# zkMIPS/zkm

Measured on AMD Instinct MI355X. Metric: segment_proofs_per_sec, higher is better.
Workload: dtype u64 (Goldilocks p = 2^64 - 2^32 + 1, integer modular)

## Files before the change

### zkm_amd/csrc/core.hip

```cpp
#include <sched.h>
#include <time.h>
#include <stdio.h>
#include <algorithm>
#include <atomic>

#include "poseidon_dev.h"
#include "zkm_internal.h"

void* zkm_ctx::alloc(size_t bytes) {
    if (bytes == 0) bytes = 8;
    void* p = nullptr;
    {
        std::lock_guard<std::mutex> g(alloc_mu);
        auto it = free_blocks.find(bytes);
        if (it != free_blocks.end()) {
            p = it->second;
            free_blocks.erase(it);
            live_blocks[p] = bytes;
            return p;
        }
    }
    zkm_ctx* const root = parent ? parent : this;
    const int ticket = root->debug_fail_allocs.load(std::memory_order_relaxed) > 0 ? root->debug_fail_allocs.fetch_sub(1) : 0;
    const bool inject = ticket > 0;
// ... 41 lines not shown
}
void zkm_ctx::drop_copy_streams() {
    hipStream_t a, b, d;
    {
        std::lock_guard<std::mutex> g(alloc_mu);
        a = copy_stream; b = copy_stream2; d = side_stream;
        copy_stream = copy_stream2 = side_stream = nullptr;
    }
    for (hipStream_t st : {a, b, d})
        if (st) { (void)hipStreamSynchronize(st); (void)hipStreamDestroy(st); }
}
static hipStream_t ensure_stream(zkm_ctx* c, hipStream_t& cs) {
    if (!cs) {
        hipStream_t st = nullptr;
        ZKM_HIP_CHECK(hipStreamCreateWithFlags(&st, hipStreamNonBlocking));
        std::lock_guard<std::mutex> g(c->alloc_mu);
        cs = st;
    }
    return cs;
}
hipStream_t zkm_ctx::ensure_copy_stream(int k) { return ensure_stream(this, k ? copy_stream2 : copy_stream); }
hipStream_t zkm_ctx::ensure_side_stream() { return ensure_stream(this, side_stream); }
void zkm_ctx::trim() {
    trim_self();
    shrink_down();
    drop_copy_streams();
    for (zkm_ctx* l : lanes) {
        l->trim_self();
        l->shrink_down();
        l->drop_copy_streams();
    }
}
static hipError_t zkm_stream_create(hipStream_t* st, int num_cus, int part_k, int part_n) {
    if (part_n > 1 && part_k >= 0 && part_k < part_n && num_cus >= 8 * part_n) {
        std::vector<uint32_t> mask((size_t)(num_cus + 31) / 32, 0);
        const int lo = (int)((long)num_cus * part_k / part_n), hi = (int)((long)num_cus * (part_k + 1) / part_n);
        for (int i = lo; i < hi; i++) mask[i / 32] |= 1u << (i % 32);
        return hipExtStreamCreateWithCUMask(st, (uint32_t)mask.size(), mask.data());
    }
    return hipStreamCreateWithFlags(st, hipStreamNonBlocking);
}
void zkm_ctx::ensure_lanes(size_t k) {
    while (lanes.size() < k) {
        zkm_ctx* l = new zkm_ctx();
        l->parent = this;
        l->device = device;
        l->num_cus = num_cus;
        l->ingest_chunk_cols = ingest_chunk_cols;
        l->keccak_parts_max_points = keccak_parts_max_points;
        l->fri_fused_division_min = fri_fused_division_min;
        l->wide_max_hashes = wide_max_hashes;
        l->leaf_mfma = leaf_mfma;
        l->quad_max_hashes = quad_max_hashes;
        l->small_ntt = small_ntt;
        l->tree_tail = tree_tail;
        l->commit_lanes = commit_lanes;
        l->max_stack = max_stack;
        l->fri_scan_combine = fri_scan_combine;
        l->pow_round_log = pow_round_log;
        l->cu_part_k = cu_part_k;
        l->cu_part_n = cu_part_n;
        hipError_t e = zkm_stream_create(&l->stream, num_cus, cu_part_k, cu_part_n);
        if (e != hipSuccess) {
            delete l;
            ZKM_HIP_CHECK(e);
        }
        lanes.push_back(l);
    }
    for (zkm_ctx* l : lanes) l->profiling = profiling;
}
void zkm_ctx::release(void* p) {
    if (!p) return;
    std::lock_guard<std::mutex> g(alloc_mu);
    auto it = live_blocks.find(p);
    if (it == live_blocks.end()) return;
    free_blocks.emplace(it->second, p);
    live_blocks.erase(it);
}
uint64_t* zkm_ctx::staging(size_t words) {
    if (words > h_staging_words) {
        if (h_staging) (void)hipHostFree(h_staging);
        size_t w = words < 4096 ? 4096 : words;
        ZKM_HIP_CHECK(hipHostMalloc((void**)&h_staging, w * sizeof(uint64_t)));
        h_staging_words = w;
    }
    return h_staging;
}
struct down_args {
    const uint32_t* src[4];
    uint32_t* dst[4];
    uint32_t words[4];
    uint32_t n;
};
__global__ __launch_bounds__(1024) void k_download(down_args a, uint64_t* flag, uint64_t seq) {
    for (uint32_t s = 0; s < a.n; s++)
        for (uint32_t i = threadIdx.x; i < a.words[s]; i += 1024) a.dst[s][i] = a.src[s][i];
    __threadfence_system();
    __syncthreads();
    if (threadIdx.x == 0) __hip_atomic_store(flag, seq, __ATOMIC_RELEASE, __HIP_MEMORY_SCOPE_SYSTEM);
}
__global__ __launch_bounds__(256) void k_download_wide(const uint4* __restrict__ src, uint4* __restrict__ dst, uint32_t n16, uint64_t* flag,
                                                       uint64_t seq, unsigned* counter) {
    for (uint32_t i = blockIdx.x * 256 + threadIdx.x; i < n16; i += gridDim.x * 256) dst[i] = src[i];
    __threadfence_system();
    __syncthreads();
    if (threadIdx.x == 0) {
// ... 257 lines not shown
        if (!out) throw std::runtime_error("zkm_ctx_create: null argument");
        int n = 0;
        ZKM_HIP_CHECK(hipGetDeviceCount(&n));
        if (device < 0 || device >= n) throw std::runtime_error("zkm_ctx_create: no such HIP device " + std::to_string(device));
        ZKM_HIP_CHECK(hipSetDevice(device));
        std::unique_ptr<zkm_ctx> c(new zkm_ctx());
        c->device = device;
        hipDeviceProp_t prop;
        ZKM_HIP_CHECK(hipGetDeviceProperties(&prop, device));
        c->num_cus = prop.multiProcessorCount;
        if (const char* part = getenv("ZKM_CU_MASK_PART")) {
            int k = -1, n = 0;
            if (sscanf(part, "%d/%d", &k, &n) == 2) { c->cu_part_k = k; c->cu_part_n = n; }
        }
        ZKM_HIP_CHECK(zkm_stream_create(&c->stream, c->num_cus, c->cu_part_k, c->cu_part_n));
        g_live_contexts.fetch_add(1, std::memory_order_relaxed);
        *out = c.release();
    });
}

void zkm_ctx_destroy(zkm_ctx* c) {
    if (!c) return;
    if (!c->parent) g_live_contexts.fetch_sub(1, std::memory_order_relaxed);
    (void)hipSetDevice(c->device);
    for (zkm_ctx* l : c->lanes) zkm_ctx_destroy(l);
    c->lanes.clear();
    (void)hipStreamSynchronize(c->stream);
    if (c->copy_stream) { (void)hipStreamSynchronize(c->copy_stream); (void)hipStreamDestroy(c->copy_stream); }
    if (c->copy_stream2) { (void)hipStreamSynchronize(c->copy_stream2); (void)hipStreamDestroy(c->copy_stream2); }
    if (c->side_stream) { (void)hipStreamSynchronize(c->side_stream); (void)hipStreamDestroy(c->side_stream); }
    for (auto& kv : c->free_blocks) (void)hipFree(kv.second);
    for (auto& kv : c->live_blocks) (void)hipFree(kv.first);
    for (auto& r : c->prof) { (void)hipEventDestroy(r.start); (void)hipEventDestroy(r.stop); }
    for (auto e : c->event_pool) (void)hipEventDestroy(e);
    if (c->h_staging) (void)hipHostFree(c->h_staging);
    if (c->h_xfer) (void)hipHostFree(c->h_xfer);
    if (c->h_down) (void)hipHostFree(c->h_down);
    if (c->block_event) (void)hipEventDestroy(c->block_event);
    (void)hipStreamDestroy(c->stream);
    delete c;
}

int zkm_ctx_set_tuning(zkm_ctx* c, const char* key, uint64_t value, char** err) {
    return zkm_api("zkm_ctx_set_tuning", err, [&] {
        if (!c || !key) throw std::runtime_error("zkm_ctx_set_tuning: null argument");
        const std::string k(key);
        auto set = [&](zkm_ctx* x) {
            if (k == "ingest_chunk_cols") x->ingest_chunk_cols = (size_t)value;
            else if (k == "keccak_parts_max_points") x->keccak_parts_max_points = (size_t)value;
            else if (k == "fri_fused_division_min") x->fri_fused_division_min = (size_t)value;
            else if (k == "wide_max_hashes") x->wide_max_hashes = (size_t)value;
            else if (k == "leaf_mfma") x->leaf_mfma = value ? 1 : 0;
            else if (k == "quad_max_hashes") x->quad_max_hashes = (size_t)value;
            else if (k == "block_after_us") x->block_after_us = value;
            else if (k == "small_ntt") x->small_ntt = value ? 1 : 0;
            else if (k == "tree_tail") x->tree_tail = value ? 1 : 0;
            else if (k == "pow_round_log") x->pow_round_log = value < 8 ? 8 : (value > 22 ? 22 : (unsigned)value);
            else if (k == "fri_scan_combine") x->fri_scan_combine = value ? 1 : 0;
            else if (k == "aux_pipeline") x->aux_pipeline = value ? 1 : 0;
            else if (k == "commit_lanes") x->commit_lanes = value < 1 ? 1 : (value > 8 ? 8 : (size_t)value);
            else if (k == "segments_memory_budget") x->segments_memory_budget = (size_t)value;
            else if (k == "max_stack") x->max_stack = value < 1 ? 1 : (value > ZKM_MAX_SEG ? ZKM_MAX_SEG : (size_t)value);
            else if (k == "throughput_profile") {
                x->commit_lanes = value ? 1 : ZKM_COMMIT_LANES;
                x->wide_max_hashes = value ? 256 : 1024;
                x->quad_max_hashes = value ? 4096 : 32768;
                x->pow_round_log = value ? 16 : 17;
            }
            else if (k == "check_ctls") x->check_ctls = value ? 1 : 0;
            else if (k == "verify") x->verify = value ? 1 : 0;
            else if (k == "boot_chain_quad") x->boot_chain_quad = value ? 1 : 0;
            else if (k == "debug_verify_flip") {
                const char* hooks = getenv("ZKM_ENABLE_TEST_HOOKS");
                if (!hooks || strcmp(hooks, "1") != 0) throw std::runtime_error("zkm_ctx_set_tuning: unknown key '" + k + "'");
                x->debug_verify_flip = value;
            }
            else if (k == "debug_ctl_key_bits") {
                const char* hooks = getenv("ZKM_ENABLE_TEST_HOOKS");
                if (!hooks || strcmp(hooks, "1") != 0) throw std::runtime_error("zkm_ctx_set_tuning: unknown key '" + k + "'");
                x->debug_ctl_key_bits = value > 128 ? 128 : (unsigned)value;
            }
            else if (k == "debug_fail_allocs") {
                const char* hooks = getenv("ZKM_ENABLE_TEST_HOOKS");
                if (!hooks || strcmp(hooks, "1") != 0) throw std::runtime_error("zkm_ctx_set_tuning: unknown key '" + k + "'");
                if (x == c) x->debug_fail_allocs.store((int)value);
            }
            else throw std::runtime_error("zkm_ctx_set_tuning: unknown key '" + k + "'");
        };
        set(c);
        for (zkm_ctx* l : c->lanes) set(l);
    });
}

uint64_t zkm_ctx_host_waits(const zkm_ctx* c) { return c ? c->host_waits : 0; }

int zkm_ctx_synchronize(zkm_ctx* c, char** err) {
    return zkm_api("zkm_ctx_synchronize", c, err, [&] { c->sync(); });
}
void* zkm_ctx_stream(zkm_ctx* c) { return c ? (void*)c->stream : nullptr; }

void zkm_ctx_memory(const zkm_ctx* c, size_t* live_bytes, size_t* cached_bytes) {
    size_t live = 0, cached = 0;
    if (c) {
        for (auto& kv : c->live_blocks) live += kv.second;
        for (auto& kv : c->free_blocks) cached += kv.first;
        for (const zkm_ctx* l : c->lanes) {
// ... 324 lines not shown
    gl_t* __restrict__ d = dst + (size_t)blockIdx.y * words;
    for (size_t i = (size_t)blockIdx.x * 256 + threadIdx.x; i < words; i += (size_t)gridDim.x * 256) d[i] = gl_canon(s[i]);
}

void zkm_launch_canon(zkm_ctx* c, gl_t* v, size_t total) {
    zkm_prof_scope ps(c, "ingest_canonicalise");
    hipLaunchKernelGGL(k_canon, dim3((total + 255) / 256), dim3(256), 0, c->stream, v, total);
    ZKM_HIP_CHECK(hipGetLastError());
}

void zkm_batch_build(zkm_batch* b, const uint64_t* src, bool src_is_values, gl_t* dev_values, const uint64_t* const* src_cols,
                     const uint64_t* const* seg_srcs) {
    zkm_ctx* c = b->ctx;
    const size_t nseg = b->nseg;
    size_t n = b->n(), N = b->N(), ncols = b->ncols * nseg;
    if (b->log_n + b->rate_bits > 30) throw std::runtime_error("polynomial batch too large");
    if (nseg == 0 || nseg > ZKM_MAX_SEG) throw std::runtime_error("polynomial batch: bad segment count");
    if (ncols > 65535 && nseg > 1) throw std::runtime_error("polynomial batch: too many stacked columns");
    if (!src && !src_cols && !seg_srcs) throw std::runtime_error("polynomial batch: no source");
    if (src_cols)
        for (size_t i = 0; i < ncols; i++)
            if (!src_cols[i]) throw std::runtime_error("polynomial batch: null column pointer");
    if (seg_srcs)
        for (size_t i = 0; i < nseg; i++)
            if (!seg_srcs[i]) throw std::runtime_error("polynomial batch: null segment pointer");
    auto copy_cols = [&](gl_t* dst, size_t c0, size_t nc, hipMemcpyKind kind, hipStream_t st) {
        if (seg_srcs) {
            for (size_t sg = 0; sg < nseg; sg++)
                ZKM_HIP_CHECK(hipMemcpyAsync(dst + sg * b->ncols * n, seg_srcs[sg], b->ncols * n * sizeof(gl_t), hipMemcpyDefault, st));
            return;
        }
        if (!src_cols) {
            ZKM_HIP_CHECK(hipMemcpyAsync(dst, src + c0 * n, nc * n * sizeof(gl_t), kind, st));
            return;
        }
        for (size_t i = 0; i < nc; i++)
            ZKM_HIP_CHECK(hipMemcpyAsync(dst + i * n, src_cols[c0 + i], n * sizeof(gl_t), hipMemcpyDefault, st));
    };
    b->coeffs = (gl_t*)c->alloc(ncols * n * sizeof(gl_t));
    b->lde = (gl_t*)c->alloc(ncols * N * sizeof(gl_t));
    b->coeff_s1 = b->rate_bits == 2 ? zkm_coeff_layout_s1(b->log_n) : 0;
    const unsigned s1 = b->coeff_s1;
    auto inverse_transform = [&](const gl_t* vals, size_t c0, size_t nc) {
        if (s1) zkm_intt_digit(c, vals, n, b->coeffs + c0 * n, n, nc, b->log_n);
        else zkm_ntt_natural_ex(c, vals, n, b->lde + c0 * N, n, b->coeffs + c0 * n, n, nc, b->log_n, true, 0);
    };
    size_t dwords = zkm_merkle_layout(b->lde_bits(), b->cap_height, b->level_off);
    b->dig_words = dwords;
    b->digests = (gl_t*)c->alloc(nseg * dwords * sizeof(gl_t));
    bool dev = !src_cols && !seg_srcs && zkm_is_device_ptr(src);
    hipMemcpyKind kind = dev ? hipMemcpyDeviceToDevice : hipMemcpyHostToDevice;
    const size_t CH = c->ingest_chunk_cols;
    bool leaves_done = false;
    if (src_is_values && !dev && nseg == 1 && CH && CH % 8 == 0 && ncols >= 2 * CH && b->log_n >= 13) {
        c->ensure_copy_stream();
        const size_t nchunks = (ncols + CH - 1) / CH;
        zkm_scratch state(c, 12 * N * sizeof(gl_t));
        std::vector<zkm_event> ev;
        ev.reserve(nchunks + 1);
        struct drain {
            zkm_ctx* c;
            ~drain() {
                (void)hipStreamSynchronize(c->copy_stream);
                (void)hipStreamSynchronize(c->stream);
            }
        } const drained{c};
        ev.emplace_back(c);
        ev[0].record(c->stream);
        ZKM_HIP_CHECK(hipStreamWaitEvent(c->copy_stream, ev[0].e, 0));
        for (size_t k = 0; k < nchunks; k++) {
            size_t c0 = k * CH, nc = std::min(CH, ncols - c0);
            gl_t* dst = dev_values ? dev_values + c0 * n : b->lde + c0 * N;
            copy_cols(dst, c0, nc, hipMemcpyHostToDevice, c->copy_stream);
            ev.emplace_back(c);
            ev.back().record(c->copy_stream);
        }
        for (size_t k = 0; k < nchunks; k++) {
            size_t c0 = k * CH, nc = std::min(CH, ncols - c0);
            gl_t* vals = dev_values ? dev_values + c0 * n : b->lde + c0 * N;
            ZKM_HIP_CHECK(hipStreamWaitEvent(c->stream, ev[k + 1].e, 0));
            if (dev_values) zkm_launch_canon(c, vals, nc * n);
            inverse_transform(vals, c0, nc);
            zkm_lde_bitrev(c, b->coeffs + c0 * n, b->lde + c0 * N, nc, b->log_n, b->rate_bits, GL_GENERATOR, s1);
            zkm_launch_merkle_leaves_chunk(c, b->lde + c0 * N, N, nc, N, state.as<gl_t>(), k == 0, k + 1 == nchunks, b->digests);
        }
        leaves_done = true;
    } else if (src_is_values && dev) {
        inverse_transform(src, 0, ncols);
    } else if (src_is_values) {
        gl_t* vals = dev_values ? dev_values : b->lde;
        bool all_dev = seg_srcs != nullptr;
        for (size_t sg = 0; all_dev && sg < nseg; sg++) all_dev = zkm_is_device_ptr(seg_srcs[sg]);
        if (all_dev && !dev_values) {
            for (size_t sg = 0; sg < nseg; sg++) inverse_transform(seg_srcs[sg], sg * b->ncols, b->ncols);
        } else if (all_dev) {
            seg_ptrs sp{};
            for (size_t sg = 0; sg < nseg; sg++) sp.p[sg] = seg_srcs[sg];
            const size_t words = b->ncols * n;
            zkm_prof_scope ps(c, "ingest_canonicalise");
            hipLaunchKernelGGL(k_gather_canon, dim3((unsigned)std::min<size_t>((words + 255) / 256, 4096), (unsigned)nseg), dim3(256), 0, c->stream, sp,
                               words, vals);
            ZKM_HIP_CHECK(hipGetLastError());
        } else {
            copy_cols(vals, 0, ncols, kind, c->stream);
            if (dev_values) zkm_launch_canon(c, vals, ncols * n);
        }
        if (!(all_dev && !dev_values)) inverse_transform(vals, 0, ncols);
    } else {
        copy_cols(b->coeffs, 0, ncols, kind, c->stream);
    }
    if (!leaves_done) {
        zkm_lde_bitrev(c, b->coeffs, b->lde, ncols, b->log_n, b->rate_bits, GL_GENERATOR, src_is_values ? s1 : 0);
        zkm_launch_merkle_leaves(c, b->lde, N, b->ncols, N, b->digests, nseg, b->lde_seg(), dwords);
    }
    if (!src_is_values && s1) {
        zkm_scratch nat(c, ncols * n * sizeof(gl_t));
        ZKM_HIP_CHECK(hipMemcpyAsync(nat.p, b->coeffs, ncols * n * sizeof(gl_t), hipMemcpyDeviceToDevice, c->stream));
        zkm_coeff_layout_convert(c, nat.as<gl_t>(), n, b->coeffs, n, ncols, b->log_n, false);
    }
    size_t capw = (size_t)4 << b->cap_height;
    b->cap.resize(nseg * capw);
    zkm_merkle_build_inner_cap(c, b->digests, b->level_off, b->lde_bits(), b->cap_height, b->cap.data(), nseg, dwords);
}

__global__ __launch_bounds__(256) void k_gather_lde_rows(const gl_t* __restrict__ lde, size_t N, unsigned lde_bits, size_t ncols,
                                                         size_t index_start, size_t step, size_t count, gl_t* __restrict__ out) {
    size_t idx = (size_t)blockIdx.x * blockDim.x + threadIdx.x;
    if (idx >= count * ncols) return;
    size_t i = idx / ncols, col = idx % ncols;
    size_t row = bitrev32((uint32_t)((index_start + i) * step), lde_bits);
    out[idx] = lde[col * N + row];
}

zkm_batch_ptr zkm_batch_new(zkm_ctx* c, size_t ncols, size_t nseg, unsigned log_n, unsigned rate_bits, unsigned cap_height) {
    if (ncols == 0) throw std::runtime_error("empty polynomial batch");
    if (cap_height > log_n + rate_bits) throw std::runtime_error("cap_height exceeds LDE size");
    zkm_batch_ptr b(new zkm_batch());
    b->ctx = c; b->ncols = ncols; b->nseg = nseg; b->log_n = log_n; b->rate_bits = rate_bits; b->cap_height = cap_height;
    return b;
}

zkm_batch* zkm_batch_commit_values_keep(zkm_ctx* c, const uint64_t* values, size_t ncols, unsigned log_n, unsigned rate_bits,
                                        unsigned cap_height, gl_t* dev_values, const uint64_t* const* columns) {
    zkm_batch_ptr b = zkm_batch_new(c, ncols, 1, log_n, rate_bits, cap_height);
    zkm_batch_build(b.get(), values, true, dev_values, columns);
    return b.release();
}

extern "C" {

int zkm_batch_commit_values(zkm_ctx* c, const uint64_t* values, size_t ncols, unsigned log_n, unsigned rate_bits,
                            unsigned cap_height, zkm_batch** out, char** err) {
    return zkm_api("zkm_batch_commit_values", c, err, [&] {
        zkm_batch_ptr b = zkm_batch_new(c, ncols, 1, log_n, rate_bits, cap_height);
        zkm_batch_build(b.get(), values, true);
        *out = b.release();
    });
}
int zkm_batch_commit_columns(zkm_ctx* c, const uint64_t* const* columns, size_t ncols, unsigned log_n, int columns_are_values,
                             unsigned rate_bits, unsigned cap_height, zkm_batch** out, char** err) {
    return zkm_api("zkm_batch_commit_columns", c, err, [&] {
        if (!columns || !out) throw std::runtime_error("zkm_batch_commit_columns: null argument");
        zkm_batch_ptr b = zkm_batch_new(c, ncols, 1, log_n, rate_bits, cap_height);
        zkm_batch_build(b.get(), nullptr, columns_are_values != 0, nullptr, columns);
        *out = b.release();
    });
}
int zkm_batch_commit_coeffs(zkm_ctx* c, const uint64_t* coeffs, size_t ncols, unsigned log_n, unsigned rate_bits,
                            unsigned cap_height, zkm_batch** out, char** err) {
    return zkm_api("zkm_batch_commit_coeffs", c, err, [&] {
        zkm_batch_ptr b = zkm_batch_new(c, ncols, 1, log_n, rate_bits, cap_height);
        zkm_batch_build(b.get(), coeffs, false);
        *out = b.release();
    });
}
// ... 237 lines not shown
```

### zkm_amd/csrc/hash.hip

```cpp
#include <atomic>
#include "poseidon_dev.h"
#include "poseidon_lat_dev.h"
#include "poseidon_mfma_dev.h"
#include "hash_constants_dev.h"
#include "zkm_internal.h"

#ifndef ZKM_LEAF_MFMA_WAVES
#define ZKM_LEAF_MFMA_WAVES (ZKM_MFMA_PARK ? 5 : 4)
#endif

#ifndef ZKM_LATENCY_PRIO
#define ZKM_LATENCY_PRIO 3
#endif
#define ZKM_RAISE_PRIO()                                              \
    do {                                                              \
        if (ZKM_LATENCY_PRIO) __builtin_amdgcn_s_setprio(ZKM_LATENCY_PRIO); \
    } while (0)

__global__ __launch_bounds__(256) void k_poseidon_permute(gl_t* states, size_t k) {
    size_t i = (size_t)blockIdx.x * blockDim.x + threadIdx.x;
    if (i >= k) return;
    uint64_t s[12];
#pragma unroll
    for (int j = 0; j < 12; j++) s[j] = states[i * 12 + j];
// ... 28 lines not shown
        c0 += k * arity; c1 += k * arity;
    }
    __device__ __forceinline__ unsigned words() const { return 2 * arity; }
    __device__ __forceinline__ uint64_t word(unsigned m) const {
        const gl_t *a = c0, *b = c1;
        return ((m & 1) ? b : a)[m >> 1];
    }
};


template <class MDS>
struct sponge_lane {
    static constexpr unsigned LANES = 1;
    static constexpr bool MFMA = std::is_same<MDS, poseidon_mds_mfma>::value;
    typedef uint64_t state_t[12];
    MDS mds;
    size_t item;
    bool live;
    __device__ __forceinline__ sponge_lane() {
        if constexpr (MFMA) {
            mds.A = poseidon_mfma_operand();
#if ZKM_MFMA_PARK
            __shared__ uint32_t park[24 * ZKM_MFMA_PARK_STRIDE];
            mds.park = park + threadIdx.x;
#endif
        }
    }
    __device__ __forceinline__ bool take(size_t n) {
        item = (size_t)blockIdx.x * blockDim.x + threadIdx.x;
        live = item < n;
        if (!MFMA && !live) return false;
        if (!live) item = n - 1;
        return true;
    }
    __device__ __forceinline__ void clear(state_t& s) const {
#pragma unroll
        for (int i = 0; i < 12; i++) s[i] = 0;
    }
    template <bool RAGGED, class Src, class I>
    __device__ __forceinline__ void load(state_t& s, const Src& src, I c, I n) const {
        if (!RAGGED) {
            uint64_t v[8];
#pragma unroll
            for (int i = 0; i < 8; i++) v[i] = src.word(c + i);
#pragma unroll
            for (int i = 0; i < 8; i++) s[i] = v[i];
        } else {
#pragma unroll
            for (int i = 0; i < 8; i++)
                if ((I)i < n - c) s[i] = src.word(c + i);
        }
    }
    __device__ __forceinline__ void permute(state_t& s, int out) const { poseidon_permute_out_t(s, out, mds); }
    template <class Src>
    __device__ __forceinline__ void copy(state_t& s, const Src& src) const {
        for (size_t c = 0; c < src.words(); c++) s[c] = src.word(c);
    }
    template <class K>
    __device__ __forceinline__ void store_digest(const state_t& s, uint64_t* digests, K k, bool on) const {
        if (!on) return;
        uint64_t* d = digests + 4 * k;
        *reinterpret_cast<ulonglong2*>(d) = make_ulonglong2(s[0], s[1]);
        *reinterpret_cast<ulonglong2*>(d + 2) = make_ulonglong2(s[2], s[3]);
    }
    __device__ __forceinline__ void load_state(state_t& s, const gl_t* __restrict__ state, size_t n) const {
#pragma unroll
        for (int i = 0; i < 12; i++) s[i] = state[(size_t)i * n + item];
    }
    __device__ __forceinline__ void store_state(const state_t& s, gl_t* __restrict__ state, size_t n) const {
        if (!live) return;
#pragma unroll
        for (int i = 0; i < 12; i++) state[(size_t)i * n + item] = s[i];
    }
};

using sponge_lane_valu = sponge_lane<poseidon_mds_valu>;
using sponge_lane_mfma = sponge_lane<poseidon_mds_mfma>;

struct sponge_quad {
    static constexpr unsigned LANES = 4;
    typedef uint64_t state_t[3];
    const poseidon_quad Q;
    const unsigned q;
    size_t item;
    bool live;
    __device__ __forceinline__ sponge_quad() : Q(threadIdx.x, table()), q(threadIdx.x & 3) {}
    static __device__ __forceinline__ const uint32_t* table() {
        __shared__ __attribute__((aligned(16))) uint32_t qtab[ZKM_QUAD_TAB_WORDS];
        quad_tab_load(qtab);
        return qtab;
    }
    __device__ __forceinline__ bool take(size_t n) {
        item = ((size_t)blockIdx.x * blockDim.x + threadIdx.x) >> 2;
        live = item < n;
        return true;
    }
    __device__ __forceinline__ void clear(state_t& s) const { s[0] = s[1] = s[2] = 0; }
    template <bool RAGGED, class Src, class I>
    __device__ __forceinline__ void load(state_t& s, const Src& src, I c, I n) const {
        if (live && (!RAGGED || c + q < n)) s[0] = src.word(c + q);
        if (live && (!RAGGED || c + 4 + q < n)) s[1] = src.word(c + 4 + q);
    }
    __device__ __forceinline__ void permute(state_t& s, int) const { poseidon_permute_quad(s, Q); }
    template <class K>
    __device__ __forceinline__ void compress(state_t& s, const uint64_t* nodes, K k, bool on) const {
        s[0] = on ? nodes[8 * k + q] : 0;
// ... 158 lines not shown

void zkm_launch_merkle_leaves_ext(zkm_ctx* c, const gl_t* c0, const gl_t* c1, size_t nleaves, unsigned arity, gl_t* digests, size_t nseg,
                                  size_t val_seg, size_t dig_seg) {
    if (arity % 4 || 2 * arity <= 4) throw std::runtime_error("merkle_leaves_ext: unsupported arity");
    if (nseg == 0 || nseg > 65535) throw std::runtime_error("merkle_leaves_ext: bad segment count");
    zkm_prof_scope ps(c, "merkle_leaves_ext");
    static constexpr decltype(&k_merkle_leaves_ext) kernel[] = {k_merkle_leaves_ext, k_merkle_leaves_ext_mfma, k_merkle_leaves_ext_quad, k_merkle_leaves_ext_wide};
    const merkle_form f = merkle_pick_form(c, nleaves * nseg, true);
    hipLaunchKernelGGL(kernel[f], leaf_grid(f, nleaves, nseg), dim3(256), 0, c->stream, c0, c1, nleaves, arity, digests, val_seg, dig_seg);
    ZKM_HIP_CHECK(hipGetLastError());
}

struct merkle_fused_args {
    const gl_t* children;
    gl_t* parents[3];
    uint32_t levels;
    size_t dig_seg;
};

__global__ __launch_bounds__(256) void k_merkle_fused(merkle_fused_args p) {
    __shared__ uint64_t sh[2][4][256];
    const unsigned tid = threadIdx.x;
    uint64_t s[12];
    {
        const ulonglong2* ch = reinterpret_cast<const ulonglong2*>(p.children + (size_t)blockIdx.z * p.dig_seg + 8 * ((size_t)blockIdx.x * 256 + tid));
        ulonglong2 a = ch[0], b = ch[1], cc = ch[2], d = ch[3];
        s[0] = a.x; s[1] = a.y; s[2] = b.x; s[3] = b.y; s[4] = cc.x; s[5] = cc.y; s[6] = d.x; s[7] = d.y;
    }
#pragma unroll 1
    for (unsigned lvl = 0; lvl < p.levels; lvl++) {
        const unsigned width = 256u >> lvl;
        if (lvl) {
#pragma unroll
            for (int w = 0; w < 4; w++) {
                s[w] = sh[(lvl - 1) & 1][w][2 * tid];
                s[4 + w] = sh[(lvl - 1) & 1][w][2 * tid + 1];
            }
        }
#pragma unroll
        for (int w = 8; w < 12; w++) s[w] = 0;
        poseidon_permute_out(s, POSEIDON_OUT_DIGEST);
        uint64_t* o = p.parents[lvl] + (size_t)blockIdx.z * p.dig_seg + 4 * ((size_t)blockIdx.x * width + tid);
        *reinterpret_cast<ulonglong2*>(o) = make_ulonglong2(s[0], s[1]);
        *reinterpret_cast<ulonglong2*>(o + 2) = make_ulonglong2(s[2], s[3]);
        if (lvl + 1 < p.levels) {
#pragma unroll
            for (int w = 0; w < 4; w++) sh[lvl & 1][w][tid] = s[w];
        }
        if (lvl + 1 == p.levels) return;
        __syncthreads();
        if (tid >= (width >> 1)) return;
    }
}

template <class Form>
__device__ __forceinline__ bool merkle_climb_level(const Form& f, unsigned slots, unsigned np, const uint64_t* in, uint64_t* out, gl_t* g, uint64_t* also = nullptr) {
    const unsigned slot = threadIdx.x / Form::LANES, wave_slot0 = (threadIdx.x >> 6) * (64 / Form::LANES);
    if (wave_slot0 >= np) return false;
    for (unsigned h0 = 0; h0 < np; h0 += slots) {
        if (h0 + wave_slot0 >= np) continue;
        const unsigned h = h0 + slot;
        const bool on = h < np;
        typename Form::state_t s;
        f.compress(s, in, h, on);
        f.store_digest(s, out, h, on);
        f.store_digest(s, g, h, on);
        if (also) f.store_digest(s, also, h, on);
    }
    return true;
}

struct merkle_fused_wide_args {
    const gl_t* children;
    gl_t* parents[6];
    uint32_t J;
    size_t dig_seg;
};
struct merkle_fused_quad_args {
    const gl_t* children;
    gl_t* parents[7];
    uint32_t J;
    size_t dig_seg;
};
template <class Form, unsigned MAXC, class Args>
__device__ __forceinline__ void merkle_fused_body(const Args& p) {
    __shared__ uint64_t sh[2][MAXC * 4];
    const unsigned tid = threadIdx.x;
    Form f;
    const unsigned C = 1u << p.J;
    const size_t seg_off = (size_t)blockIdx.z * p.dig_seg;
    {
        const gl_t* src = p.children + seg_off + (size_t)blockIdx.x * C * 4;
        for (unsigned w = tid; w < C * 4; w += 256) sh[0][w] = src[w];
    }
    __syncthreads();
    for (unsigned lvl = 0; lvl < p.J; lvl++) {
        const unsigned np = C >> (lvl + 1);
        if (!merkle_climb_level(f, 256 / Form::LANES, np, sh[lvl & 1], sh[(lvl + 1) & 1], p.parents[lvl] + seg_off + (size_t)blockIdx.x * np * 4))
            return;
        __syncthreads();
    }
}
__global__ __launch_bounds__(256) void k_merkle_fused_wide(merkle_fused_wide_args p) {
    ZKM_RAISE_PRIO();
    merkle_fused_body<sponge_wide, 64>(p);
}
// ... 41 lines not shown
    __syncthreads();
    if (tid == 0) {
        const unsigned ticket = atomicAdd(p.counter, 1u);
        if (ticket == gridDim.x * gridDim.z - 1) {
            *p.counter = 0;
            __threadfence_system();
            __hip_atomic_store(p.flag, p.seq, __ATOMIC_RELEASE, __HIP_MEMORY_SCOPE_SYSTEM);
        }
    }
}
bool zkm_merkle_tail(zkm_ctx* c, gl_t* digests, const std::vector<size_t>& level_off, unsigned log_leaves, unsigned cap_height, uint64_t* cap_out,
                     unsigned l0, size_t nseg, size_t dig_seg) {
    const unsigned J = log_leaves - l0 - cap_height;
    if (!c->tree_tail || J == 0 || J > 11 || cap_height > 6) return false;
    if (merkle_pick_form(c, (size_t)1 << (log_leaves - l0 - 1), false) == MERKLE_LANE) return false;
    const size_t tail_lds = (((size_t)1 << J) * 4 + ((size_t)1 << J) * 2) * sizeof(uint64_t);
    static std::atomic<uint64_t> lds_ok{0};
    if (tail_lds + ZKM_QUAD_TAB_WORDS * sizeof(uint32_t) > 64 * 1024 &&
        zkm_allow_big_lds(c, (const void*)k_merkle_tail, lds_ok, 128 * 1024) != hipSuccess)
        return false;
    merkle_tail_args a{};
    a.children = digests + level_off[l0];
    for (unsigned k = 0; k < J; k++) a.parents[k] = digests + level_off[l0 + 1 + k];
    a.J = J;
    a.dig_seg = dig_seg;
    a.wide_np_max = c->wide_max_hashes ? 16 : 0;
    const size_t capw = ((size_t)4 << cap_height) * nseg;
    const uint64_t seq = c->xfer_begin(capw * 8, &a.host_cap, &a.flag, &a.counter);
    a.seq = seq;
    const size_t C = (size_t)1 << J;
    unsigned threads = (unsigned)(C >> 1) * 4;
    if (threads > 256) threads = 256;
    if (threads < 64) threads = 64;
    {
        zkm_prof_scope ps(c, "merkle_compress");
        hipLaunchKernelGGL(k_merkle_tail, dim3(1u << cap_height, 1, (unsigned)nseg), dim3(threads), tail_lds, c->stream, a);
        ZKM_HIP_CHECK(hipGetLastError());
    }
    c->xfer_finish(seq, cap_out, capw * 8);
    return true;
}

size_t zkm_merkle_layout(unsigned log_leaves, unsigned cap_height, std::vector<size_t>& level_off) {
    if (cap_height > log_leaves) throw std::runtime_error("cap_height exceeds tree height");
    level_off.clear();
    size_t total = 0;
    for (unsigned l = 0; l + cap_height <= log_leaves; l++) {
        level_off.push_back(total);
        total += ((size_t)1 << (log_leaves - l)) * 4;
    }
    return total;
}

void zkm_merkle_build_inner(zkm_ctx* c, gl_t* digests, const std::vector<size_t>& level_off, unsigned log_leaves,
                            unsigned cap_height, size_t nseg, size_t dig_seg) {
    const unsigned top = log_leaves - cap_height;
    const unsigned z = (unsigned)nseg;
    unsigned l = 0;
    while (l < top) {
        zkm_prof_scope ps(c, "merkle_compress");
        const unsigned log_p1 = log_leaves - l - 1;
        const unsigned rem = top - l;
        const size_t p1 = (size_t)1 << log_p1, h1 = p1 * nseg;
        merkle_form form = merkle_pick_form(c, h1, false);
        if (form == MERKLE_LANE && log_p1 < 8) form = MERKLE_QUAD;
        if (form == MERKLE_LANE) {
            merkle_fused_args a{};
            a.dig_seg = dig_seg;
            a.children = digests + level_off[l];
            a.levels = rem < 3 ? rem : 3;
            for (unsigned k = 0; k < a.levels; k++) a.parents[k] = digests + level_off[l + 1 + k];
            hipLaunchKernelGGL(k_merkle_fused, dim3((unsigned)(((size_t)1 << log_p1) / 256), 1, z), dim3(256), 0, c->stream, a);
            l += a.levels;
        } else if (form == MERKLE_WIDE) {
            merkle_fused_wide_args a{};
            a.dig_seg = dig_seg;
            a.children = digests + level_off[l];
            unsigned J = rem < 6 ? rem : 6;
            if (J > log_p1 + 1) J = log_p1 + 1;
            a.J = J;
            for (unsigned k = 0; k < J; k++) a.parents[k] = digests + level_off[l + 1 + k];
            hipLaunchKernelGGL(k_merkle_fused_wide, dim3((unsigned)(((size_t)2 << log_p1) >> J), 1, z), dim3(256), 0, c->stream, a);
            l += J;
        } else {
            merkle_fused_quad_args a{};
            a.dig_seg = dig_seg;
            a.children = digests + level_off[l];
            unsigned J = 1;
            while (J < rem && J < 7 && J <= log_p1 && merkle_pick_form(c, h1 >> J, false) != MERKLE_WIDE) J++;
            a.J = J;
            for (unsigned k = 0; k < J; k++) a.parents[k] = digests + level_off[l + 1 + k];
            hipLaunchKernelGGL(k_merkle_fused_quad, dim3((unsigned)(((size_t)2 << log_p1) >> J), 1, z), dim3(256), 0, c->stream, a);
            l += J;
        }
        ZKM_HIP_CHECK(hipGetLastError());
    }
}

static void download_caps(zkm_ctx* c, const gl_t* digests, size_t cap_off, unsigned cap_height, uint64_t* cap_out, size_t nseg, size_t dig_seg) {
    const size_t capw = (size_t)4 << cap_height;
    if (nseg == 1) {
        c->download(cap_out, digests + cap_off, capw * sizeof(uint64_t));
        return;
    }
    zkm_scratch tmp(c, nseg * capw * sizeof(gl_t));
    ZKM_HIP_CHECK(hipMemcpy2DAsync(tmp.p, capw * sizeof(gl_t), digests + cap_off, dig_seg * sizeof(gl_t), capw * sizeof(gl_t), nseg,
                                   hipMemcpyDeviceToDevice, c->stream));
    c->download(cap_out, tmp.p, nseg * capw * sizeof(uint64_t));
}

void zkm_merkle_build_inner_cap(zkm_ctx* c, gl_t* digests, const std::vector<size_t>& level_off, unsigned log_leaves, unsigned cap_height,
                                uint64_t* cap_out, size_t nseg, size_t dig_seg) {
    const unsigned TAIL_LOG = 11;
    if (c->tree_tail && log_leaves <= 24 && log_leaves >= cap_height + 1) {
        const unsigned l0 = log_leaves > TAIL_LOG ? log_leaves - TAIL_LOG : 0;
        if (log_leaves - l0 > cap_height) {
            if (l0) zkm_merkle_build_inner(c, digests, level_off, log_leaves, log_leaves - l0, nseg, dig_seg);
            if (zkm_merkle_tail(c, digests, level_off, log_leaves, cap_height, cap_out, l0, nseg, dig_seg)) return;
            if (l0) {
                std::vector<size_t> rest(level_off.begin() + l0, level_off.end());
                zkm_merkle_build_inner(c, digests, rest, log_leaves - l0, cap_height, nseg, dig_seg);
                download_caps(c, digests, level_off[log_leaves - cap_height], cap_height, cap_out, nseg, dig_seg);
                return;
            }
        }
    }
    zkm_merkle_build_inner(c, digests, level_off, log_leaves, cap_height, nseg, dig_seg);
    download_caps(c, digests, level_off[log_leaves - cap_height], cap_height, cap_out, nseg, dig_seg);
}

struct __attribute__((aligned(8))) keccak_pair { uint64_t x, y; };

__global__ __launch_bounds__(256) void k_keccakf(uint64_t* __restrict__ states, size_t k) {
    const size_t idx = (size_t)blockIdx.x * blockDim.x + threadIdx.x;
    if (idx >= k) return;
    uint64_t a[25];
    uint64_t* st = states + idx * 25;
#pragma unroll
    for (int i = 0; i < 12; i++) {
        const keccak_pair v = *reinterpret_cast<const keccak_pair*>(st + 2 * i);
        a[2 * i] = v.x;
        a[2 * i + 1] = v.y;
    }
    a[24] = st[24];
    keccakf_dev(a);
#pragma unroll
    for (int i = 0; i < 12; i++) *reinterpret_cast<keccak_pair*>(st + 2 * i) = keccak_pair{a[2 * i], a[2 * i + 1]};
    st[24] = a[24];
}

void zkm_launch_keccakf(zkm_ctx* c, uint64_t* states, size_t k) {
    if (!k) return;
    zkm_prof_scope ps(c, "keccakf");
    hipLaunchKernelGGL(k_keccakf, dim3((k + 255) / 256), dim3(256), 0, c->stream, states, k);
    ZKM_HIP_CHECK(hipGetLastError());
}

enum {
    PROBE_PERMUTE_LANE = ZKM_POSEIDON_PROBE_PERMUTE_LANE, PROBE_PERMUTE_LANE_MFMA = ZKM_POSEIDON_PROBE_PERMUTE_LANE_MFMA,
    PROBE_PERMUTE_QUAD = ZKM_POSEIDON_PROBE_PERMUTE_QUAD, PROBE_PERMUTE_WIDE = ZKM_POSEIDON_PROBE_PERMUTE_WIDE,
    PROBE_MDS_VALU = ZKM_POSEIDON_PROBE_MDS_VALU, PROBE_MDS_MFMA = ZKM_POSEIDON_PROBE_MDS_MFMA, PROBE_MDS_QUAD = ZKM_POSEIDON_PROBE_MDS_QUAD,
    PROBE_MDS_ROWS = ZKM_POSEIDON_PROBE_MDS_ROWS, PROBE_GROUP3 = ZKM_POSEIDON_PROBE_GROUP3, PROBE_GROUP3_QUAD = ZKM_POSEIDON_PROBE_GROUP3_QUAD,
    PROBE_GROUP2 = ZKM_POSEIDON_PROBE_GROUP2, PROBE_FOLD = ZKM_POSEIDON_PROBE_FOLD, PROBE_FOLD_TY = ZKM_POSEIDON_PROBE_FOLD_TY,
    PROBE_SBOX7 = ZKM_POSEIDON_PROBE_SBOX7, PROBE_SBOX_DELTA = ZKM_POSEIDON_PROBE_SBOX_DELTA, PROBE_ADD_RC0 = ZKM_POSEIDON_PROBE_ADD_RC0
};
static_assert(POSEIDON_OUT_ALL == ZKM_POSEIDON_OUT_ALL && POSEIDON_OUT_CAPACITY == ZKM_POSEIDON_OUT_CAPACITY && POSEIDON_OUT_DIGEST == ZKM_POSEIDON_OUT_DIGEST,
              "include/zkm_hip.h names the output modes of poseidon_dev.h");

template <class Form, int PROBE>
__device__ __forceinline__ void poseidon_probe_lane_body(const uint64_t* __restrict__ in, size_t n, uint64_t* __restrict__ out, unsigned arg) {
    Form f;
    if (!f.take(n)) return;
    typename Form::state_t s;
#pragma unroll
    for (int i = 0; i < 12; i++) s[i] = in[f.item * 12 + i];
    if constexpr (PROBE == PROBE_PERMUTE_LANE || PROBE == PROBE_PERMUTE_LANE_MFMA) {
        f.permute(s, (int)arg);
    } else if constexpr (PROBE == PROBE_MDS_VALU || PROBE == PROBE_MDS_MFMA) {
        f.mds.layer(s, (int)arg);
    } else if constexpr (PROBE == PROBE_MDS_ROWS) {
// ... 119 lines not shown
```

### zkm_amd/csrc/zkm_internal.h

```cpp
#pragma once
#include <hip/hip_runtime.h>
#include <stdint.h>
#include <stdlib.h>
#include <string.h>

#include <algorithm>
#include <atomic>
#include <exception>
#include <map>
#include <memory>
#include <mutex>
#include <tuple>
#include <type_traits>
#include <stdexcept>
#include <string>
#include <initializer_list>
#include <vector>

#include "../../include/zkm_hip.h"
#include "gl_dev.h"
#include "proof_blob.h"
#include "tables.h"

#define ZKM_HIP_CHECK(expr)                                                                                  \
    do {                                                                                                     \
        hipError_t _e = (expr);                                                                              \
        if (_e != hipSuccess)                                                                                \
            throw std::runtime_error(std::string(#expr) + ": " + hipGetErrorString(_e) + " (" + __FILE__ + ":" + \
                                     std::to_string(__LINE__) + ")");                                        \
    } while (0)

struct zkm_segment_error : std::runtime_error {
    size_t seg;
    zkm_segment_error(size_t s, const char* msg) : std::runtime_error(msg), seg(s) {}
};

struct zkm_prof_rec {
    const char* name;
    hipEvent_t start, stop;
};

#ifndef ZKM_MAX_SEG
#define ZKM_MAX_SEG 32
#endif
struct seg_gl { gl_t v[ZKM_MAX_SEG]; };
struct seg_gl2 { gl_t v[2 * ZKM_MAX_SEG]; };

#ifndef ZKM_COMMIT_LANES
#define ZKM_COMMIT_LANES 4
#endif
#ifndef ZKM_LEAF_MFMA_DEFAULT
#define ZKM_LEAF_MFMA_DEFAULT 1
#endif

template <class A> struct zkm_seg_args { A v[ZKM_MAX_SEG]; };

struct zkm_twiddles {
    gl_t* fwd = nullptr;
    gl_t* inv = nullptr;
    unsigned log_max = 0;
};

struct zkm_ctx {
    int device = 0;
    hipStream_t stream = nullptr;
    hipStream_t copy_stream = nullptr;
    hipStream_t copy_stream2 = nullptr;
    hipStream_t side_stream = nullptr;
    int boot_chain_quad = 0;
    size_t ingest_chunk_cols = 32;
    size_t keccak_parts_max_points = (size_t)1 << 15;
    size_t fri_fused_division_min = ~(size_t)0;
    int fri_scan_combine = 1;
    size_t small_ntt = 1;
    unsigned pow_round_log = 17;
    int aux_pipeline = 1;
    size_t commit_lanes = ZKM_COMMIT_LANES;
    size_t segments_memory_budget = 0;
    size_t last_stack = 0;
    size_t prev_stack = 0;
    size_t max_stack = ZKM_MAX_SEG;
    int leaf_mfma = ZKM_LEAF_MFMA_DEFAULT;
    size_t wide_max_hashes = 1024;
    size_t quad_max_hashes = 32768;
    int num_cus = 256;
    int cu_part_k = -1, cu_part_n = 0;
    bool profiling = false;
    std::vector<zkm_prof_rec> prof;
    std::vector<hipEvent_t> event_pool;
    struct agg { const char* name; uint64_t launches; double ms; };
    std::vector<agg> prof_agg;
    bool prof_agg_valid = false;
    std::multimap<size_t, void*> free_blocks;
    std::map<void*, size_t> live_blocks;
    std::mutex alloc_mu;
    zkm_ctx* parent = nullptr;
    std::atomic<int> debug_fail_allocs{0};
    int check_ctls = 0;
    unsigned debug_ctl_key_bits = 0;
    int verify = 0;
    uint64_t debug_verify_flip = 0;
    zkm_twiddles tw;
    std::map<std::pair<uint64_t, unsigned>, gl_t*> pow_tables;
    std::map<std::tuple<uint64_t, unsigned, unsigned>, gl_t*> lde_ct_tables;
    size_t resident_bytes = 0;
    uint64_t* h_staging = nullptr;
    size_t h_staging_words = 0;
    std::vector<zkm_ctx*> lanes;
    void ensure_lanes(size_t k);

    void* alloc(size_t bytes);
    void release(void* p);
    void trim_self();
    void trim();
    void drop_copy_streams();
    hipStream_t ensure_copy_stream(int k = 0);
    hipStream_t ensure_side_stream();
    void shrink_down();
    void ensure_twiddles(unsigned log_n);
    const gl_t* pow_table(uint64_t shift, unsigned log_n);
    uint64_t* staging(size_t words);
    struct xfer { void* dst; const void* src; size_t bytes; };
    void download(std::initializer_list<xfer> xs);
    void download(void* dst, const void* src, size_t bytes) { download({xfer{dst, src, bytes}}); }
    void upload(void* dst, const void* src, size_t bytes);
    char* h_xfer = nullptr;
    uint64_t down_seq = 0;
    void wait_flag(const uint64_t* flag, uint64_t seq);
    uint64_t block_after_us = 50;
    hipEvent_t block_event = nullptr;
    uint64_t blocked_waits = 0;
    void ensure_xfer();
    uint64_t xfer_begin(size_t bytes, uint64_t** host_slot, uint64_t** flag, unsigned** counter);
    void xfer_finish(uint64_t seq, void* dst, size_t bytes);
    unsigned* d_counter = nullptr;
    unsigned long long* d_pow_best = nullptr;
    unsigned long long* pow_best();
// ... 141 lines not shown
    unsigned coeff_s1 = 0;
    gl_t* lde = nullptr;
    gl_t* digests = nullptr;
    size_t dig_words = 0;
    std::vector<size_t> level_off;
    std::vector<uint64_t> cap;
    size_t coeff_seg() const { return ncols << log_n; }
    size_t lde_seg() const { return ncols << (log_n + rate_bits); }
    size_t n() const { return (size_t)1 << log_n; }
    size_t N() const { return (size_t)1 << (log_n + rate_bits); }
    unsigned lde_bits() const { return log_n + rate_bits; }
    unsigned top() const { return lde_bits() - cap_height; }
};

struct zkm_batch_deleter {
    void operator()(zkm_batch* b) const { zkm_batch_free(b); }
};
using zkm_batch_ptr = std::unique_ptr<zkm_batch, zkm_batch_deleter>;
zkm_batch_ptr zkm_batch_new(zkm_ctx* c, size_t ncols, size_t nseg, unsigned log_n, unsigned rate_bits, unsigned cap_height);

inline bool zkm_is_device_ptr(const void* p) {
    hipPointerAttribute_t a;
    hipError_t e = hipPointerGetAttributes(&a, p);
    if (e != hipSuccess) {
        (void)hipGetLastError();
        return false;
    }
    return a.type == hipMemoryTypeDevice;
}

template <class A, class... X>
void zkm_launch_segs(hipStream_t stream, void (*kernel)(zkm_seg_args<A>, X...), const A* segs, size_t nseg, size_t grid_x, unsigned threads, X... x) {
    static_assert(sizeof(zkm_seg_args<A>) + sizeof...(X) * 8 <= 3840, "the descriptors travel as kernel arguments (4 KiB)");
    if (nseg == 0 || nseg > ZKM_MAX_SEG) throw std::runtime_error("zkm_launch_segs: segment count out of range");
    if (!grid_x) return;
    zkm_seg_args<A> S{};
    std::copy(segs, segs + nseg, S.v);
    hipLaunchKernelGGL(kernel, dim3((unsigned)grid_x, 1, (unsigned)nseg), dim3(threads), 0, stream, S, x...);
    ZKM_HIP_CHECK(hipGetLastError());
}

void zkm_launch_poseidon_permute(zkm_ctx*, gl_t* states, size_t k);
void zkm_launch_mul_selftest_branchfree(zkm_ctx*, const uint64_t* a, const uint64_t* b, size_t n, uint64_t* out);
void zkm_launch_keccakf(zkm_ctx*, uint64_t* states, size_t k);
void zkm_launch_merkle_leaves(zkm_ctx*, const gl_t* lde, size_t nrows, size_t ncols, size_t col_stride, gl_t* digests, size_t nseg = 1,
                              size_t lde_seg = 0, size_t dig_seg = 0);
void zkm_launch_merkle_leaves_chunk(zkm_ctx*, const gl_t* lde, size_t nrows, size_t nc, size_t col_stride, gl_t* state, bool first,
                                    bool last, gl_t* digests);
void zkm_ntt_natural_ex(zkm_ctx* c, const gl_t* in, size_t cs_in, gl_t* scratch, size_t cs_s, gl_t* out, size_t cs_out, size_t ncols,
                        unsigned log_n, bool inverse, uint64_t shift);
void zkm_launch_merkle_leaves_ext(zkm_ctx*, const gl_t* c0, const gl_t* c1, size_t nleaves, unsigned arity, gl_t* digests, size_t nseg = 1,
                                  size_t val_seg = 0, size_t dig_seg = 0);
size_t zkm_merkle_layout(unsigned log_leaves, unsigned cap_height, std::vector<size_t>& level_off);
void zkm_merkle_build_inner(zkm_ctx*, gl_t* digests, const std::vector<size_t>& level_off, unsigned log_leaves, unsigned cap_height,
                            size_t nseg = 1, size_t dig_seg = 0);
void zkm_merkle_build_inner_cap(zkm_ctx*, gl_t* digests, const std::vector<size_t>& level_off, unsigned log_leaves, unsigned cap_height,
                                uint64_t* cap_out, size_t nseg = 1, size_t dig_seg = 0);
bool zkm_merkle_tail(zkm_ctx*, gl_t* digests, const std::vector<size_t>& level_off, unsigned log_leaves, unsigned cap_height, uint64_t* cap_out,
                     unsigned l0, size_t nseg = 1, size_t dig_seg = 0);

void zkm_ntt_dif_bitrev(zkm_ctx*, gl_t* data, size_t ncols, size_t col_stride, unsigned log_n, bool inverse);
void zkm_ntt_natural(zkm_ctx*, gl_t* in_scratch, gl_t* out, size_t ncols, size_t col_stride_in, size_t col_stride_out,
                     unsigned log_n, bool inverse, uint64_t shift);
void zkm_launch_scale_pad(zkm_ctx*, const gl_t* in, size_t col_stride_in, gl_t* out, size_t col_stride_out, size_t ncols,
                          unsigned log_n_in, unsigned log_n_out, uint64_t shift);
void zkm_lde_bitrev(zkm_ctx*, const gl_t* coeffs, gl_t* out, size_t ncols, unsigned log_n, unsigned rate_bits, uint64_t shift,
                    unsigned coeff_s1 = 0);
inline unsigned zkm_coeff_layout_s1(unsigned log_n) { return (log_n >= 18 && log_n <= 20) ? log_n - 12 : 0; }
GL_HD uint32_t zkm_coeff_exponent(uint32_t P, unsigned s1) {
    if (!s1) return P;
    const uint32_t t_hi = P & ((1u << s1) - 1), cc = (P >> s1) & ((1u << (12 - s1)) - 1), blk = P >> 12;
    return (t_hi << 12) | (cc << s1) | bitrev32(blk, s1);
}
void zkm_intt_digit(zkm_ctx*, const gl_t* values, size_t cs_in, gl_t* coeffs, size_t cs_out, size_t ncols, unsigned log_n);
void zkm_coeff_layout_convert(zkm_ctx*, const gl_t* in, size_t cs_in, gl_t* out, size_t cs_out, size_t ncols, unsigned log_n, bool to_natural);

int zkm_live_contexts();
void zkm_batch_build(zkm_batch* b, const uint64_t* src, bool src_is_values, gl_t* dev_values = nullptr,
                     const uint64_t* const* src_cols = nullptr, const uint64_t* const* seg_srcs = nullptr);
zkm_batch* zkm_batch_commit_values_keep(zkm_ctx* c, const uint64_t* values, size_t ncols, unsigned log_n, unsigned rate_bits,
                                        unsigned cap_height, gl_t* dev_values, const uint64_t* const* columns = nullptr);
void zkm_prove_single_table_aux(zkm_ctx* c, int table_id, const zkm_stark_config* cfg, size_t ncols, unsigned log_n, const zkm_batch* trace_batch,
                                const zkm_batch* aux_batch, size_t naux_ctl, const zkm_ctl_table* table, const zkm_ctl_z* zs,
                                const uint32_t* colset_ids, size_t nzs, const uint64_t* lookup_challenges, const std::vector<zkm_challenger*>& chs,
                                const std::vector<uint64_t*>& proofs);
void zkm_launch_canon(zkm_ctx* c, gl_t* v, size_t total);
void zkm_host_poseidon_permute(uint64_t st[12]);
void zkm_host_poseidon_permute_reference(uint64_t st[12]);
const zkm_table_lookup* zkm_table_lookups(int table_id, size_t* n);
void zkm_table_lookup_columns_device(zkm_ctx* c, int table_id, const uint64_t* challenges, size_t nch, const gl_t* d_trace, size_t n,
                                     gl_t* d_out, size_t nseg = 1, size_t trace_seg = 0, size_t out_seg = 0);
struct zkm_writer_seg {
    const void* in[4];
    size_t k, n, aux;
    gl_t* out;
    int* bad;
    void* tmp[2];
};
void zkm_launch_writers(zkm_ctx* c, int table_id, const zkm_writer_seg* segs, size_t nseg);

struct zkm_memory_job {
    zkm_ctx* c;
    const char* what;
    const uint64_t* d_ops;
    size_t nops;
    zkm_scratch small, keys_a, keys_b, idx_a, idx_b, start;
    unsigned long long* d_acc = nullptr;
    uint64_t* d_count = nullptr;
    const uint32_t* idx = nullptr;
    uint64_t M = 0, count = 0;
// ... 84 lines not shown
```

Baseline: 16.89.

## Add per-level Merkle kernels and fuse narrow leaf hashing into first level

Adds one-level-per-launch Merkle compression kernels (VALU and MFMA variants) used when a level has at least level_min_hashes hashes, replacing the lane/quad form for large levels. It also extends the tree-tail split so those wide levels run level by level. For matrices with at most four columns, leaf hashing is skipped: leaves are copied straight from the LDE as digests and the first tree level is compressed in the same kernel, saving a launch and a pass over the leaf digests. This adds a new tuning knob, and the wider-level path may be slower than the existing fused climb kernels.

```diff
diff --git a/zkm_amd/csrc/core.hip b/zkm_amd/csrc/core.hip
--- a/zkm_amd/csrc/core.hip
+++ b/zkm_amd/csrc/core.hip
@@ -117,6 +117,7 @@
         l->wide_max_hashes = wide_max_hashes;
         l->leaf_mfma = leaf_mfma;
         l->quad_max_hashes = quad_max_hashes;
+        l->level_min_hashes = level_min_hashes;
         l->small_ntt = small_ntt;
         l->tree_tail = tree_tail;
         l->commit_lanes = commit_lanes;
@@ -480,6 +481,7 @@
             else if (k == "wide_max_hashes") x->wide_max_hashes = (size_t)value;
             else if (k == "leaf_mfma") x->leaf_mfma = value ? 1 : 0;
             else if (k == "quad_max_hashes") x->quad_max_hashes = (size_t)value;
+            else if (k == "level_min_hashes") x->level_min_hashes = (size_t)value;
             else if (k == "block_after_us") x->block_after_us = value;
             else if (k == "small_ntt") x->small_ntt = value ? 1 : 0;
             else if (k == "tree_tail") x->tree_tail = value ? 1 : 0;
@@ -910,6 +912,7 @@
     hipMemcpyKind kind = dev ? hipMemcpyDeviceToDevice : hipMemcpyHostToDevice;
     const size_t CH = c->ingest_chunk_cols;
     bool leaves_done = false;
+    zkm_leaf_matrix leaf_rows{};
     if (src_is_values && !dev && nseg == 1 && CH && CH % 8 == 0 && ncols >= 2 * CH && b->log_n >= 13) {
         c->ensure_copy_stream();
         const size_t nchunks = (ncols + CH - 1) / CH;
@@ -969,7 +972,8 @@
     }
     if (!leaves_done) {
         zkm_lde_bitrev(c, b->coeffs, b->lde, ncols, b->log_n, b->rate_bits, GL_GENERATOR, src_is_values ? s1 : 0);
-        zkm_launch_merkle_leaves(c, b->lde, N, b->ncols, N, b->digests, nseg, b->lde_seg(), dwords);
+        if (b->ncols <= 4) leaf_rows = zkm_leaf_matrix{b->lde, b->ncols, N, b->lde_seg()};
+        else zkm_launch_merkle_leaves(c, b->lde, N, b->ncols, N, b->digests, nseg, b->lde_seg(), dwords);
     }
     if (!src_is_values && s1) {
         zkm_scratch nat(c, ncols * n * sizeof(gl_t));
@@ -978,7 +982,7 @@
     }
     size_t capw = (size_t)4 << b->cap_height;
     b->cap.resize(nseg * capw);
-    zkm_merkle_build_inner_cap(c, b->digests, b->level_off, b->lde_bits(), b->cap_height, b->cap.data(), nseg, dwords);
+    zkm_merkle_build_inner_cap(c, b->digests, b->level_off, b->lde_bits(), b->cap_height, b->cap.data(), nseg, dwords, leaf_rows.lde ? &leaf_rows : nullptr);
 }
 
 __global__ __launch_bounds__(256) void k_gather_lde_rows(const gl_t* __restrict__ lde, size_t N, unsigned lde_bits, size_t ncols,
diff --git a/zkm_amd/csrc/hash.hip b/zkm_amd/csrc/hash.hip
--- a/zkm_amd/csrc/hash.hip
+++ b/zkm_amd/csrc/hash.hip
@@ -104,6 +104,18 @@
         }
     }
     __device__ __forceinline__ void permute(state_t& s, int out) const { poseidon_permute_out_t(s, out, mds); }
+    __device__ __forceinline__ void two_to_one(state_t& s) const {
+#pragma unroll
+        for (int i = 8; i < 12; i++) s[i] = 0;
+        permute(s, POSEIDON_OUT_DIGEST);
+    }
+    template <class K>
+    __device__ __forceinline__ void compress(state_t& s, const uint64_t* nodes, K k, bool) const {
+        const ulonglong2* ch = reinterpret_cast<const ulonglong2*>(nodes + 8 * k);
+        const ulonglong2 a = ch[0], b = ch[1], cc = ch[2], d = ch[3];
+        s[0] = a.x; s[1] = a.y; s[2] = b.x; s[3] = b.y; s[4] = cc.x; s[5] = cc.y; s[6] = d.x; s[7] = d.y;
+        two_to_one(s);
+    }
     template <class Src>
     __device__ __forceinline__ void copy(state_t& s, const Src& src) const {
         for (size_t c = 0; c < src.words(); c++) s[c] = src.word(c);
@@ -368,6 +380,55 @@
         if (tid >= (width >> 1)) return;
     }
 }
+
+template <class Form>
+__device__ __forceinline__ void merkle_level_body(const gl_t* __restrict__ children, gl_t* __restrict__ parents, size_t nparents, size_t dig_seg) {
+    Form f;
+    if (!f.take(nparents)) return;
+    const size_t seg_off = (size_t)blockIdx.z * dig_seg;
+    typename Form::state_t s;
+    f.compress(s, children + seg_off, f.item, f.live);
+    f.store_digest(s, parents + seg_off, f.item, f.live);
+}
+template <class Form>
+__device__ __forceinline__ void merkle_level_cols_body(leaf_cols src, size_t nparents, gl_t* __restrict__ leaves, gl_t* __restrict__ parents, size_t dig_seg) {
+    Form f;
+    if (!f.take(nparents)) return;
+    src.seek(2 * f.item);
+    const size_t seg_off = (size_t)blockIdx.z * dig_seg;
+    typename Form::state_t s;
+#pragma unroll
+    for (int m = 0; m < 4; m++) {
+        ulonglong2 v = make_ulonglong2(0, 0);
+        if ((size_t)m < src.ncols) v = *reinterpret_cast<const ulonglong2*>(src.lde + m * src.col_stride);
+        s[m] = v.x;
+        s[4 + m] = v.y;
+    }
+    if (f.live) {
+        ulonglong2* lv = reinterpret_cast<ulonglong2*>(leaves + seg_off + 8 * f.item);
+#pragma unroll
+        for (int m = 0; m < 4; m++) lv[m] = make_ulonglong2(s[2 * m], s[2 * m + 1]);
+    }
+    f.two_to_one(s);
+    f.store_digest(s, parents + seg_off, f.item, f.live);
+}
+__global__ __launch_bounds__(256) void k_merkle_level(const gl_t* __restrict__ children, gl_t* __restrict__ parents, size_t nparents, size_t dig_seg) {
+    merkle_level_body<sponge_lane_valu>(children, parents, nparents, dig_seg);
+}
+__global__ __launch_bounds__(256) ZKM_LEAF_MFMA_ATTR void k_merkle_level_mfma(const gl_t* __restrict__ children, gl_t* __restrict__ parents, size_t nparents,
+                                                                             size_t dig_seg) {
+    merkle_level_body<sponge_lane_mfma>(children, parents, nparents, dig_seg);
+}
+__global__ __launch_bounds__(256) void k_merkle_level_cols(const gl_t* __restrict__ lde, size_t nparents, size_t ncols, size_t col_stride,
+                                                           gl_t* __restrict__ leaves, gl_t* __restrict__ parents, size_t lde_seg, size_t dig_seg) {
+    merkle_level_cols_body<sponge_lane_valu>(leaf_cols{lde, ncols, col_stride, lde_seg}, nparents, leaves, parents, dig_seg);
+}
+__global__ __launch_bounds__(256) ZKM_LEAF_MFMA_ATTR void k_merkle_level_cols_mfma(const gl_t* __restrict__ lde, size_t nparents, size_t ncols, size_t col_stride,
+                                                                                  gl_t* __restrict__ leaves, gl_t* __restrict__ parents, size_t lde_seg,
+                                                                                  size_t dig_seg) {
+    merkle_level_cols_body<sponge_lane_mfma>(leaf_cols{lde, ncols, col_stride, lde_seg}, nparents, leaves, parents, dig_seg);
+}
+static bool merkle_level_launch(const zkm_ctx* c, size_t hashes) { return c->level_min_hashes && hashes >= c->level_min_hashes; }
 
 template <class Form>
 __device__ __forceinline__ bool merkle_climb_level(const Form& f, unsigned slots, unsigned np, const uint64_t* in, uint64_t* out, gl_t* g, uint64_t* also = nullptr) {
@@ -515,16 +576,35 @@
     return total;
 }
 
+static bool merkle_narrow_first_level(const zkm_ctx* c, const zkm_leaf_matrix& m, unsigned log_leaves, unsigned cap_height, size_t nseg) {
+    return m.ncols <= 4 && log_leaves > cap_height && merkle_level_launch(c, ((size_t)1 << (log_leaves - 1)) * nseg) &&
+           m.col_stride % 2 == 0 && m.seg % 2 == 0 && (uintptr_t)m.lde % 16 == 0;
+}
 void zkm_merkle_build_inner(zkm_ctx* c, gl_t* digests, const std::vector<size_t>& level_off, unsigned log_leaves,
-                            unsigned cap_height, size_t nseg, size_t dig_seg) {
+                            unsigned cap_height, size_t nseg, size_t dig_seg, const zkm_leaf_matrix* narrow) {
     const unsigned top = log_leaves - cap_height;
     const unsigned z = (unsigned)nseg;
+    if (narrow && !merkle_narrow_first_level(c, *narrow, log_leaves, cap_height, nseg))
+        throw std::logic_error("merkle_build_inner: the first level of this tree is not a column launch");
     unsigned l = 0;
     while (l < top) {
         zkm_prof_scope ps(c, "merkle_compress");
         const unsigned log_p1 = log_leaves - l - 1;
         const unsigned rem = top - l;
         const size_t p1 = (size_t)1 << log_p1, h1 = p1 * nseg;
+        if (merkle_level_launch(c, h1)) {
+            const dim3 grid = leaf_grid(MERKLE_LANE, p1, nseg);
+            gl_t* const parents = digests + level_off[l + 1];
+            if (narrow && l == 0)
+                hipLaunchKernelGGL(c->leaf_mfma ? k_merkle_level_cols_mfma : k_merkle_level_cols, grid, dim3(256), 0, c->stream, narrow->lde, p1,
+                                   narrow->ncols, narrow->col_stride, digests + level_off[0], parents, narrow->seg, dig_seg);
+            else
+                hipLaunchKernelGGL(c->leaf_mfma ? k_merkle_level_mfma : k_merkle_level, grid, dim3(256), 0, c->stream, digests + level_off[l], parents, p1,
+                                   dig_seg);
+            ZKM_HIP_CHECK(hipGetLastError());
+            l++;
+            continue;
+        }
         merkle_form form = merkle_pick_form(c, h1, false);
         if (form == MERKLE_LANE && log_p1 < 8) form = MERKLE_QUAD;
         if (form == MERKLE_LANE) {
@@ -573,12 +653,17 @@
 }
 
 void zkm_merkle_build_inner_cap(zkm_ctx* c, gl_t* digests, const std::vector<size_t>& level_off, unsigned log_leaves, unsigned cap_height,
-                                uint64_t* cap_out, size_t nseg, size_t dig_seg) {
+                                uint64_t* cap_out, size_t nseg, size_t dig_seg, const zkm_leaf_matrix* narrow) {
+    if (narrow && !merkle_narrow_first_level(c, *narrow, log_leaves, cap_height, nseg)) {
+        zkm_launch_merkle_leaves(c, narrow->lde, (size_t)1 << log_leaves, narrow->ncols, narrow->col_stride, digests, nseg, narrow->seg, dig_seg);
+        narrow = nullptr;
+    }
     const unsigned TAIL_LOG = 11;
     if (c->tree_tail && log_leaves <= 24 && log_leaves >= cap_height + 1) {
-        const unsigned l0 = log_leaves > TAIL_LOG ? log_leaves - TAIL_LOG : 0;
+        unsigned l0 = log_leaves > TAIL_LOG ? log_leaves - TAIL_LOG : 0;
+        while (l0 + cap_height < log_leaves && merkle_level_launch(c, ((size_t)1 << (log_leaves - l0 - 1)) * nseg)) l0++;
         if (log_leaves - l0 > cap_height) {
-            if (l0) zkm_merkle_build_inner(c, digests, level_off, log_leaves, log_leaves - l0, nseg, dig_seg);
+            if (l0) zkm_merkle_build_inner(c, digests, level_off, log_leaves, log_leaves - l0, nseg, dig_seg, narrow);
             if (zkm_merkle_tail(c, digests, level_off, log_leaves, cap_height, cap_out, l0, nseg, dig_seg)) return;
             if (l0) {
                 std::vector<size_t> rest(level_off.begin() + l0, level_off.end());
@@ -588,7 +673,7 @@
             }
         }
     }
-    zkm_merkle_build_inner(c, digests, level_off, log_leaves, cap_height, nseg, dig_seg);
+    zkm_merkle_build_inner(c, digests, level_off, log_leaves, cap_height, nseg, dig_seg, narrow);
     download_caps(c, digests, level_off[log_leaves - cap_height], cap_height, cap_out, nseg, dig_seg);
 }
 
diff --git a/zkm_amd/csrc/zkm_internal.h b/zkm_amd/csrc/zkm_internal.h
--- a/zkm_amd/csrc/zkm_internal.h
+++ b/zkm_amd/csrc/zkm_internal.h
@@ -51,6 +51,9 @@
 #endif
 #ifndef ZKM_LEAF_MFMA_DEFAULT
 #define ZKM_LEAF_MFMA_DEFAULT 1
+#endif
+#ifndef ZKM_LEVEL_MIN_HASHES
+#define ZKM_LEVEL_MIN_HASHES ((size_t)1 << 16)
 #endif
 
 template <class A> struct zkm_seg_args { A v[ZKM_MAX_SEG]; };
@@ -83,6 +86,7 @@
     int leaf_mfma = ZKM_LEAF_MFMA_DEFAULT;
     size_t wide_max_hashes = 1024;
     size_t quad_max_hashes = 32768;
+    size_t level_min_hashes = ZKM_LEVEL_MIN_HASHES;
     int num_cus = 256;
     int cu_part_k = -1, cu_part_n = 0;
     bool profiling = false;
@@ -330,10 +334,11 @@
 void zkm_launch_merkle_leaves_ext(zkm_ctx*, const gl_t* c0, const gl_t* c1, size_t nleaves, unsigned arity, gl_t* digests, size_t nseg = 1,
                                   size_t val_seg = 0, size_t dig_seg = 0);
 size_t zkm_merkle_layout(unsigned log_leaves, unsigned cap_height, std::vector<size_t>& level_off);
+struct zkm_leaf_matrix { const gl_t* lde; size_t ncols, col_stride, seg; };
 void zkm_merkle_build_inner(zkm_ctx*, gl_t* digests, const std::vector<size_t>& level_off, unsigned log_leaves, unsigned cap_height,
-                            size_t nseg = 1, size_t dig_seg = 0);
+                            size_t nseg = 1, size_t dig_seg = 0, const zkm_leaf_matrix* narrow = nullptr);
 void zkm_merkle_build_inner_cap(zkm_ctx*, gl_t* digests, const std::vector<size_t>& level_off, unsigned log_leaves, unsigned cap_height,
-                                uint64_t* cap_out, size_t nseg = 1, size_t dig_seg = 0);
+                                uint64_t* cap_out, size_t nseg = 1, size_t dig_seg = 0, const zkm_leaf_matrix* narrow = nullptr);
 bool zkm_merkle_tail(zkm_ctx*, gl_t* digests, const std::vector<size_t>& level_off, unsigned log_leaves, unsigned cap_height, uint64_t* cap_out,
                      unsigned l0, size_t nseg = 1, size_t dig_seg = 0);
 
```

New measurement: 17.01, median of 6. Within noise of the previous version (+0.7%).
